# zyc-123/InstanceDiff

Measured on AMD Instinct MI355X. Metric: denoising steps/sec (256x256 bs16), higher is better.
Workload: dtype f32; 1 GPU; 256x256 1-ch synthetic, 1000-step reverse chain, batch 16 per GPU, 2 UNet fwd + reverse update per step; global_batch=16, parallelism=replicas x1 (no collective)

## Files before the change

instancediff_amd/csrc/conv_args.h:

```cpp
#pragma once
#include "common.h"

namespace idiff_detail {

struct GnTail {
    const float* gamma;
    const float* beta;
    const float* film;
    long long film_ld;
    float eps;
    int groups;
    float* out_a;
    float* out_b;
    float* mean_rstd;
};

struct ConvArgs {
    const float* src0;
    const float* src1;
    long long bs0, bs1;
    int C0v, C1v;
    int C0r;
    int Cin;
    int B, Hin, Win, Hout, Wout;
    int Cout;
    const float* wpk;
    const float* wwino;
    const float* wwino4;
    const float* bias;
    const float* pro_a;
    const float* pro_b;
    float* out;
    long long obs;
    const float* res;
    long long rbs;
    const float* vec;
    const float* aux;
    long long abs_;
    const float* aux_a;
    const float* aux_b;
    float* stats;
    GnTail gn;
    int tiles_x, ntiles, ncob;
    unsigned total_wg;
};

bool conv_wino_eligible(const ConvArgs& a, int ks, int mode);
int launch_conv_wino(const ConvArgs& a, int mode, hipStream_t st);

long long conv_wino4_items(const ConvArgs& a, int ks, int mode, bool requested = false);
int launch_conv_wino4(const ConvArgs& a, int mode, hipStream_t st);
int launch_conv_wino4h(const ConvArgs& a, int mode, hipStream_t st);

bool conv1x1_x3_eligible(const ConvArgs& a, int mode);
int launch_conv1x1_x3(const ConvArgs& a, int mode, const void* wx3, hipStream_t st);

bool conv_bf16_eligible(const ConvArgs& a, int ks, int mode, const void* wbf16);
int launch_conv_bf16(const ConvArgs& a, int mode, const void* wbf16, hipStream_t st);

}
```

instancediff_amd/csrc/conv_igemm.hip:

```cpp
#include <stdlib.h>

#include <type_traits>

#include "conv_args.h"

using idiff_detail::ConvArgs;

namespace {

typedef float floatx2 __attribute__((ext_vector_type(2)));

template <int KS, int CK, int TWL, int MODE, bool VECW, int MB, int SPEC>
__global__ __launch_bounds__(256) void conv_igemm_kernel(const ConvArgs a) {
    constexpr int BM = 32 * MB;
    constexpr int TW = 1 << TWL;
    constexpr int TH = 256 / TW;
    constexpr int PAD = KS / 2;
    constexpr int TRH = TH + KS - 1;
    constexpr int RS = TW + KS - 1;
    constexpr int PS = TRH * RS;
    constexpr int IN_TILE = ((CK * PS + 3) / 4) * 4;
    constexpr int TAPS = KS * KS;
    constexpr int W_TILE = TAPS * CK * BM;
    constexpr int BUF = IN_TILE + W_TILE;
// ... 466 lines not shown
        if (KS == 3 && MODE == IDIFF_CONV_NORMAL && MB == 2 && vecw) {
            if (a.pro_a) return launch_conv<KS, CK, 5, MODE, true, MB, 2>(a, st);
            if (a.src1) return launch_conv<KS, CK, 5, MODE, true, MB, 3>(a, st);
            return launch_conv<KS, CK, 5, MODE, true, MB, 1>(a, st);
        }
        return vecw ? launch_conv<KS, CK, 5, MODE, true, MB, 0>(a, st) : launch_conv<KS, CK, 5, MODE, false, MB, 0>(a, st);
    }
    if (twl == 4) return vecw ? launch_conv<KS, CK, 4, MODE, true, MB, 0>(a, st) : launch_conv<KS, CK, 4, MODE, false, MB, 0>(a, st);
    return vecw ? launch_conv<KS, CK, 3, MODE, true, MB, 0>(a, st) : launch_conv<KS, CK, 3, MODE, false, MB, 0>(a, st);
}

template <int KS, int CK, int MODE>
int dispatch_mb(const ConvArgs& a, int twl, int mb, bool vecw, hipStream_t st) {
    return mb == 2 ? dispatch_tw<KS, CK, MODE, 2>(a, twl, vecw, st) : dispatch_tw<KS, CK, MODE, 1>(a, twl, vecw, st);
}

inline int pick_twl(int Wout) { return Wout >= 24 ? 5 : (Wout >= 16 ? 4 : 3); }

__global__ void pack_weight_kernel(const float* __restrict__ w, float* __restrict__ out, int Cout, int Cin, int taps, int transpose) {
    const long long n = (long long)Cout * Cin * taps;
    for (long long i = blockIdx.x * (long long)blockDim.x + threadIdx.x; i < n; i += (long long)gridDim.x * blockDim.x) {
        if (!transpose) {
            const int co = i % Cout;
            const int ci = (i / Cout) % Cin;
            const int tap = i / ((long long)Cout * Cin);
            out[i] = w[((long long)co * Cin + ci) * taps + tap];
        } else {
            const int ci = i % Cin;
            const int co = (i / Cin) % Cout;
            const int tap = i / ((long long)Cout * Cin);
            out[i] = w[((long long)co * Cin + ci) * taps + (taps - 1 - tap)];
        }
    }
}

}

static thread_local int g_last_algo = IDIFF_CONV_ALGO_DIRECT;
extern "C" int idiff_conv2d_last_algo(void) { return g_last_algo; }

extern "C" int idiff_conv2d_num_tiles(int Hout, int Wout) {
    const int twl = pick_twl(Wout);
    const int TW = 1 << twl, TH = 256 / TW;
    return ((Wout + TW - 1) / TW) * ((Hout + TH - 1) / TH);
}

static int conv2d_run(const idiff_conv_desc* d, idiff_stream_t stream, const bool plan) {
    IDIFF_CHECK_ARG(d && d->src0 && d->wpk && d->out, "conv2d: null pointer");
    IDIFF_CHECK_ARG(d->B > 0 && d->C0 > 0 && d->Cout > 0 && d->Hin > 0 && d->Win > 0, "conv2d: bad dims");
    IDIFF_CHECK_ARG(d->ks == 1 || d->ks == 3 || d->ks == 7, "conv2d: ks must be 1, 3 or 7 (got %d)", d->ks);
    IDIFF_CHECK_ARG(d->mode >= 0 && d->mode <= 2, "conv2d: bad mode %d", d->mode);
    IDIFF_CHECK_ARG((d->C1 > 0) == (d->src1 != nullptr), "conv2d: src1/C1 mismatch");
    IDIFF_CHECK_ARG(!(d->pro_a && d->C1 > 0), "conv2d: prologue needs a single source");
    IDIFF_CHECK_ARG((d->pro_a == nullptr) == (d->pro_b == nullptr), "conv2d: pro_a/pro_b must both be set");
    IDIFF_CHECK_ARG(!d->aux || (d->aux_a && d->aux_b), "conv2d: aux needs aux_a/aux_b");
    ConvArgs a;
    a.src0 = d->src0;
    a.src1 = d->src1;
    a.bs0 = d->src0_bstride;
    a.bs1 = d->src1_bstride;
    a.B = d->B;
    a.C0r = d->C0;
    a.Hin = d->Hin;
    a.Win = d->Win;
    a.Cout = d->Cout;
    a.wpk = d->wpk;
    a.wwino = d->wwino;
    a.wwino4 = d->wwino4;
    a.bias = d->bias;
    a.pro_a = d->pro_a;
    a.pro_b = d->pro_b;
    a.out = d->out;
    a.obs = d->out_bstride;
    a.res = d->res;
    a.rbs = d->res_bstride;
    a.vec = d->vec;
    a.aux = d->aux;
    a.abs_ = d->aux_bstride;
    a.aux_a = d->aux_a;
    a.aux_b = d->aux_b;
    a.stats = d->stats;
    memset(&a.gn, 0, sizeof(a.gn));
    const bool want_gn = d->gn_out_a != nullptr;
    if (want_gn) {
        IDIFF_CHECK_ARG(d->stats && d->gn_out_b && d->gn_groups > 0 && d->Cout % d->gn_groups == 0 && d->Cout / d->gn_groups <= 256,
                        "conv2d: GroupNorm finalize needs stats, gn_out_b and groups dividing Cout (<= 256 channels per group)");
        a.gn.gamma = d->gn_gamma, a.gn.beta = d->gn_beta, a.gn.film = d->gn_film, a.gn.film_ld = d->gn_film_ld, a.gn.eps = d->gn_eps;
        a.gn.groups = d->gn_groups, a.gn.out_a = d->gn_out_a, a.gn.out_b = d->gn_out_b, a.gn.mean_rstd = d->gn_mean_rstd;
    }
    auto finalize_after = [&](int rc) -> int {
        if (rc != IDIFF_OK || !want_gn) return rc;
        return idiff_gn_finalize(d->stats, a.ntiles, a.B, a.Cout, d->gn_groups, a.Hout * a.Wout, d->gn_gamma, d->gn_beta, d->gn_film, d->gn_film_ld,
                                 d->gn_eps, d->gn_out_a, d->gn_out_b, d->gn_mean_rstd, stream);
    };
    if (d->mode == IDIFF_CONV_UNSHUFFLE2) {
        IDIFF_CHECK_ARG(d->ks == 1 && d->C1 == 0, "conv2d: unshuffle mode needs ks=1 and a single source");
        IDIFF_CHECK_ARG(d->Hin % 2 == 0 && d->Win % 2 == 0, "conv2d: unshuffle needs even H, W");
        a.C0v = d->C0 * 4;
        a.C1v = 0;
        a.Hout = d->Hin / 2;
        a.Wout = d->Win / 2;
    } else if (d->mode == IDIFF_CONV_UPSAMPLE2) {
        a.C0v = d->C0;
        a.C1v = d->C1;
        a.Hout = d->Hin * 2;
        a.Wout = d->Win * 2;
    } else {
        a.C0v = d->C0;
        a.C1v = d->C1;
        a.Hout = d->Hin;
        a.Wout = d->Win;
    }
    a.Cin = a.C0v + a.C1v;
    IDIFF_CHECK_ARG(a.bs0 >= (long long)d->C0 * d->Hin * d->Win, "conv2d: src0_bstride too small");
    IDIFF_CHECK_ARG(d->C1 == 0 || a.bs1 >= (long long)d->C1 * d->Hin * d->Win, "conv2d: src1_bstride too small");
    IDIFF_CHECK_ARG(a.obs >= (long long)d->Cout * a.Hout * a.Wout, "conv2d: out_bstride too small");
    int twl = pick_twl(a.Wout);
    const int mb = a.Cout <= 32 ? 1 : 2;
    const bool vecw = (a.Cout % 4 == 0) && ((reinterpret_cast<uintptr_t>(a.wpk) & 15) == 0);
    const bool in16 = (reinterpret_cast<uintptr_t>(a.src0) & 15) == 0 && (reinterpret_cast<uintptr_t>(a.src1) & 15) == 0 && a.bs0 % 4 == 0 &&
                      (!a.src1 || a.bs1 % 4 == 0);
    if (d->ks == 1 && d->mode == IDIFF_CONV_NORMAL && !a.stats && mb == 2 && vecw && in16 && ((long long)a.Hout * a.Wout) % 256 == 0 &&
        a.Wout >= 32) {
        a.Win = a.Wout = a.Hout * a.Wout;
        a.Hin = a.Hout = 1;
        twl = 8;
    }
    const int TW = 1 << twl, TH = 256 / TW;
    const int bm = 32 * mb;
    a.tiles_x = (a.Wout + TW - 1) / TW;
    a.ntiles = a.tiles_x * ((a.Hout + TH - 1) / TH);
    a.ncob = (a.Cout + bm - 1) / bm;
    const long long total = (long long)a.B * a.ntiles * a.ncob;
    IDIFF_CHECK_ARG(total < (1ll << 31), "conv2d: grid too large");
    a.total_wg = (unsigned)total;
    hipStream_t st = (hipStream_t)stream;
    const bool hard = d->algo_request > 0;
    const int req = (hard ? d->algo_request : -d->algo_request) - 1;
    IDIFF_CHECK_ARG(req == -1 || req == IDIFF_CONV_ALGO_DIRECT || req == IDIFF_CONV_ALGO_WINOGRAD || req == IDIFF_CONV_ALGO_WINOGRAD4 ||
                        req == IDIFF_CONV_ALGO_WINOGRAD4H || req == IDIFF_CONV_ALGO_X3 || req == IDIFF_CONV_ALGO_BF16,
                    "conv2d: bad algo_request %d", d->algo_request);
    IDIFF_CHECK_ARG(d->operands == 0 || d->operands == 1, "conv2d: bad operands %d", d->operands);
    {
        const bool reqbf = req == IDIFF_CONV_ALGO_BF16;
        const bool can = idiff_detail::conv_bf16_eligible(a, d->ks, d->mode, d->wbf16);
        IDIFF_CHECK_ARG(!(hard && reqbf) || can, "conv2d: algo_request bf16 but the layer is not a 3x3 that tiles for it (Cout %% 64, C0 / C1 %% 32, "
                        "Hout %% 8, Wout %% 32) or has no bf16 image");
        if (can && (reqbf || (req == -1 && d->operands == 1))) {
            g_last_algo = IDIFF_CONV_ALGO_BF16;
            if (plan) return IDIFF_OK;
            return finalize_after(idiff_detail::launch_conv_bf16(a, d->mode, d->wbf16, st));
        }
    }
    {
        static const bool x3_on = [] {
            const char* e = getenv("IDIFF_X3");
            return !e || atoi(e) != 0;
        }();
        const bool reqx3 = req == IDIFF_CONV_ALGO_X3;
        bool can = false;
        ConvArgs ax = a;
        if (d->ks == 1 && d->wx3 != nullptr && (reinterpret_cast<uintptr_t>(d->wx3) & 15) == 0) {
            if (d->mode == IDIFF_CONV_NORMAL) {
                can = twl == 8 && idiff_detail::conv1x1_x3_eligible(ax, d->mode);
            } else if (d->mode == IDIFF_CONV_UNSHUFFLE2) {
                ax.ncob = a.Cout / 64;
                ax.ntiles = (int)(((long long)a.Hout * a.Wout) / 256);
                ax.tiles_x = ax.ntiles;
                const long long tot = (long long)a.B * ax.ntiles * ax.ncob;
                ax.total_wg = (unsigned)tot;
                can = tot > 0 && tot < (1ll << 31) && idiff_detail::conv1x1_x3_eligible(ax, d->mode);
            }
        }
        IDIFF_CHECK_ARG(!(hard && reqx3) || can, "conv2d: algo_request bf16x3 but the layer is not a 1x1 that tiles by 256 pixels with a split weight image");
        if (can && (reqx3 || (req == -1 && x3_on))) {
            g_last_algo = IDIFF_CONV_ALGO_X3;
            if (plan) return IDIFF_OK;
            return idiff_detail::launch_conv1x1_x3(ax, d->mode, d->wx3, st);
        }
    }
    static const int w4h_mode = [] {
        const char* e = getenv("IDIFF_W4H");
        return e ? atoi(e) : 1;
    }();
    const bool req4 = req == IDIFF_CONV_ALGO_WINOGRAD4, req4h = req == IDIFF_CONV_ALGO_WINOGRAD4H;
    const long long items16 = (req == -1 || req4 || req4h) ? idiff_detail::conv_wino4_items(a, d->ks, d->mode, req4 || req4h) : 0;
    if (items16 > 0) {
        const long long items8 = (long long)a.ntiles * a.ncob;
        const bool w4_ok = a.Cin >= 16;
        IDIFF_CHECK_ARG(!(hard && req4) || w4_ok, "conv2d: algo_request F(4x4,3x3) 16x32-item kernel needs Cin >= 16 (got %d)", a.Cin);
        bool half;
        if (req4h) half = true;
        else if (req4 && w4_ok) half = false;
        else if (items16 >= 16 && w4_ok) half = w4h_mode == 2 || (w4h_mode == 3 && a.src1 != nullptr);
        else half = w4h_mode >= 1 && items8 >= 16;
        if (half) {
            g_last_algo = IDIFF_CONV_ALGO_WINOGRAD4H;
            if (plan) return IDIFF_OK;
            return finalize_after(idiff_detail::launch_conv_wino4h(a, d->mode, st));
        }
        if (w4_ok && (req4 || items16 >= 16)) {
            g_last_algo = IDIFF_CONV_ALGO_WINOGRAD4;
            if (plan) return IDIFF_OK;
            return finalize_after(idiff_detail::launch_conv_wino4(a, d->mode, st));
        }
    }
    IDIFF_CHECK_ARG(!hard || !(req4 || req4h), "conv2d: algo_request F(4x4,3x3) but the shape does not tile for it");
    if ((req == -1 || req == IDIFF_CONV_ALGO_WINOGRAD || !hard) && req != IDIFF_CONV_ALGO_DIRECT && idiff_detail::conv_wino_eligible(a, d->ks, d->mode)) {
        g_last_algo = IDIFF_CONV_ALGO_WINOGRAD;
        if (plan) return IDIFF_OK;
        return finalize_after(idiff_detail::launch_conv_wino(a, d->mode, st));
    }
    IDIFF_CHECK_ARG(!hard || req != IDIFF_CONV_ALGO_WINOGRAD, "conv2d: algo_request F(2x2,3x3) but the shape does not tile for it");
    g_last_algo = IDIFF_CONV_ALGO_DIRECT;
    if (plan) {
        IDIFF_CHECK_ARG(!(d->ks == 1 && d->mode == IDIFF_CONV_UPSAMPLE2), "conv2d: upsample mode needs ks=3");
        IDIFF_CHECK_ARG(d->ks != 7 || d->mode == IDIFF_CONV_NORMAL, "conv2d: ks=7 needs normal mode");
        return IDIFF_OK;
    }
    if (d->ks == 3) {
        if (d->mode == IDIFF_CONV_NORMAL) return finalize_after(dispatch_mb<3, 8, IDIFF_CONV_NORMAL>(a, twl, mb, vecw, st));
        return finalize_after(dispatch_mb<3, 8, IDIFF_CONV_UPSAMPLE2>(a, twl, mb, vecw, st));
    }
    if (d->ks == 1) {
        IDIFF_CHECK_ARG(d->mode != IDIFF_CONV_UPSAMPLE2, "conv2d: upsample mode needs ks=3");
        if (d->mode == IDIFF_CONV_NORMAL) return finalize_after(dispatch_mb<1, 16, IDIFF_CONV_NORMAL>(a, twl, mb, vecw, st));
        return finalize_after(dispatch_mb<1, 16, IDIFF_CONV_UNSHUFFLE2>(a, twl, mb, vecw, st));
    }
    IDIFF_CHECK_ARG(d->mode == IDIFF_CONV_NORMAL, "conv2d: ks=7 needs normal mode");
    return finalize_after(dispatch_mb<7, 2, IDIFF_CONV_NORMAL>(a, twl, mb, vecw, st));
}

extern "C" int idiff_conv2d_fwd(const idiff_conv_desc* d, idiff_stream_t stream) { return conv2d_run(d, stream, false); }

extern "C" int idiff_conv2d_plan(const idiff_conv_desc* d) {
    const int keep = g_last_algo;
    const int rc = conv2d_run(d, nullptr, true);
    const int algo = g_last_algo;
    g_last_algo = keep;
    return rc != IDIFF_OK ? rc : algo;
}

static int pack_common(const float* w, float* wpk, int Cout, int Cin, int ks, int tr, idiff_stream_t stream) {
    IDIFF_CHECK_ARG(w && wpk && Cout > 0 && Cin > 0 && ks > 0, "pack_conv_weight: bad args");
    const long long n = (long long)Cout * Cin * ks * ks;
    const int grid = (int)((n + 255) / 256 > 4096 ? 4096 : (n + 255) / 256);
    hipLaunchKernelGGL(pack_weight_kernel, dim3(grid), dim3(256), 0, (hipStream_t)stream, w, wpk, Cout, Cin, ks * ks, tr);
    IDIFF_CHECK_LAUNCH("pack_conv_weight");
    return IDIFF_OK;
}
extern "C" int idiff_pack_conv_weight(const float* w, float* wpk, int Cout, int Cin, int ks, idiff_stream_t stream) {
    return pack_common(w, wpk, Cout, Cin, ks, 0, stream);
}
extern "C" int idiff_pack_conv_weight_T(const float* w, float* wpk, int Cout, int Cin, int ks, idiff_stream_t stream) {
    return pack_common(w, wpk, Cout, Cin, ks, 1, stream);
}
```

instancediff_amd/ops.py:

```python
import contextlib
import ctypes as C
import math
import os
import threading

import torch

from . import _lib
from ._lib import ConvDesc, check

CONV_NORMAL, CONV_UPSAMPLE2, CONV_UNSHUFFLE2 = 0, 1, 2
ACT_NONE, ACT_SILU, ACT_GELU = 0, 1, 2
SDE_STEP, SDE_MEAN, SDE_ODE = 0, 1, 2

PROFILE = None
ALGO_TRACE = None
WGRAD_TRACE = None


def launch_count():
    return int(_lib.load().idiff_launch_count())


def _stream():
    return C.c_void_p(torch.cuda.current_stream().cuda_stream)


def _p(t):
    return None if t is None else C.c_void_p(t.data_ptr())


def _chk(t, name="tensor", dtype=torch.float32):
    if t is None:
        return
    if not t.is_cuda:
        raise _lib.IdiffError(f"{name} must live on the GPU (the hot path has no CPU fallback)")
    if t.dtype != dtype:
        raise _lib.IdiffError(f"{name} must be {dtype}, got {t.dtype}")


def _bs(t, name="tensor"):
    _chk(t, name)
    exp = 1
    for d in range(t.dim() - 1, 0, -1):
        if t.shape[d] != 1 and t.stride(d) != exp:
            raise _lib.IdiffError(f"{name}: samples must be contiguous (shape {tuple(t.shape)}, strides {t.stride()})")
        exp *= t.shape[d]
    return t.stride(0) if t.shape[0] > 1 else max(exp, t.stride(0))


def _c(t, name="tensor", dtype=torch.float32):
    _chk(t, name, dtype)
    if t is not None and not t.is_contiguous():
        raise _lib.IdiffError(f"{name} must be contiguous")
    return t


WINOGRAD = bool(int(os.environ.get("IDIFF_WINOGRAD", "1")))
X3 = bool(int(os.environ.get("IDIFF_X3", "1")))
WINOGRAD4 = WINOGRAD and bool(int(os.environ.get("IDIFF_WINOGRAD4", "1")))
WINOGRAD4_DGRAD = bool(int(os.environ.get("IDIFF_WINOGRAD4_DGRAD", "1")))


CONV_ALGO_DIRECT, CONV_ALGO_WINOGRAD, CONV_ALGO_STREAM1X1, CONV_ALGO_WINOGRAD4, CONV_ALGO_WINOGRAD4H, CONV_ALGO_X3 = 0, 1, 2, 3, 4, 5
CONV_ALGO_BF16 = 6
_ALGO_REQUEST = threading.local()
CONV_OPERANDS = ("f32", "bf16")
_OPERANDS = threading.local()


@contextlib.contextmanager
def conv_operands(kind):
    if kind not in CONV_OPERANDS:
        raise ValueError(f"conv operands must be one of {CONV_OPERANDS}, got {kind!r}")
    old = getattr(_OPERANDS, "kind", "f32")
    _OPERANDS.kind = kind
    try:
        yield
    finally:
        _OPERANDS.kind = old


def current_conv_operands():
    return getattr(_OPERANDS, "kind", "f32")


@contextlib.contextmanager
def request_conv3x3_algo(algo):
    old = getattr(_ALGO_REQUEST, "algo", None)
    _ALGO_REQUEST.algo = algo
    try:
        yield
    finally:
        _ALGO_REQUEST.algo = old


def _alloc_conv_images(w, transpose, bf16=False):
    lib = _lib.load()
    _c(w, "weight")
    co, ci, k, _ = w.shape
    out = torch.empty((k * k, co, ci) if transpose else (k * k, ci, co), device=w.device, dtype=torch.float32)
    if bf16 and k == 3:
        out.bf16 = torch.empty((lib.idiff_conv_weight_bf16_bytes(co, ci, 1 if transpose else 0) // 2,), device=w.device, dtype=torch.int16)
    if k == 3 and WINOGRAD and co % 8 == 0 and ci % 8 == 0 and (ci if transpose else co) % 16 == 0:
        cconv, kconv = (ci, co) if transpose else (co, ci)
        out.wino = torch.empty((16 * kconv * ((cconv + 63) // 64) * 64,), device=w.device, dtype=torch.float32)
        if WINOGRAD4 and (WINOGRAD4_DGRAD or not transpose):
            out.wino4 = torch.empty((36 * kconv * ((cconv + 63) // 64) * 64,), device=w.device, dtype=torch.float32)
    cconv1, kconv1 = (ci, co) if transpose else (co, ci)
    if k == 1 and X3 and cconv1 % 64 == 0 and kconv1 >= 32 and kconv1 % 8 == 0:
        out.x3 = torch.empty((lib.idiff_conv1x1_x3_image_bytes(cconv1, kconv1) // 2,), device=w.device, dtype=torch.int16)
    return out


def _fill_conv_images(out, w, transpose, algo=None):
    lib = _lib.load()
    co, ci, k, _ = w.shape
    tr = 1 if transpose else 0
    if algo is None or algo == CONV_ALGO_DIRECT:
        fn = lib.idiff_pack_conv_weight_T if transpose else lib.idiff_pack_conv_weight
        check(fn(_p(w), _p(out), co, ci, k, _stream()), "pack_conv_weight")
    if hasattr(out, "wino") and (algo is None or algo == CONV_ALGO_WINOGRAD):
        check(lib.idiff_pack_conv_weight_wino(_p(w), _p(out.wino), co, ci, tr, _stream()), "pack_conv_weight_wino")
    if hasattr(out, "wino4") and (algo is None or algo in (CONV_ALGO_WINOGRAD4, CONV_ALGO_WINOGRAD4H)):
        check(lib.idiff_pack_conv_weight_wino4(_p(w), _p(out.wino4), co, ci, tr, _stream()), "pack_conv_weight_wino4")
    if hasattr(out, "x3") and (algo is None or algo == CONV_ALGO_X3):
        cconv1, kconv1 = (ci, co) if transpose else (co, ci)
        wm = w.reshape(co, ci).t().contiguous() if transpose else w
        check(lib.idiff_pack_conv1x1_x3(_p(wm), out.x3.data_ptr(), cconv1, kconv1, _stream()), "pack_conv1x1_x3")
    if hasattr(out, "bf16") and (algo is None or algo == CONV_ALGO_BF16):
        check(lib.idiff_pack_conv_weight_bf16(_p(w), out.bf16.data_ptr(), co, ci, tr, _stream()), "pack_conv_weight_bf16")


def pack_conv_weight(w, transpose=False, bf16=False):
    out = _alloc_conv_images(w, transpose, bf16)
    _fill_conv_images(out, w, transpose)
    return out


class LazyConvWeight:

    def __init__(self, w, transpose=False):
        self.w, self.transpose = _c(w, "weight"), transpose


def conv2d(src0, wpk, bias, ks, Cout, src1=None, mode=CONV_NORMAL, pro=None, out=None, res=None, vec=None, aux=None,
           want_stats=False, algo=None, gn=None, operands=None):
    lib = _lib.load()
    B, C0, Hin, Win = src0.shape
    operands = current_conv_operands() if operands is None else operands
    if operands not in CONV_OPERANDS:
        raise ValueError(f"conv operands must be one of {CONV_OPERANDS}, got {operands!r}")
    bf16 = operands == "bf16" and ks == 3
    lazy = wpk if isinstance(wpk, LazyConvWeight) else None
    if lazy is not None:
        wpk = _alloc_conv_images(lazy.w, lazy.transpose, bf16 or algo == CONV_ALGO_BF16)
    d = ConvDesc()
    if bf16:
        d.operands = 1
    wb = getattr(wpk, "bf16", None)
    if wb is not None and ks == 3:
        d.wbf16 = wb.data_ptr()
    if algo is not None:
        d.algo_request = 1 + algo
    elif ks == 3 and getattr(_ALGO_REQUEST, "algo", None) is not None:
        d.algo_request = -(1 + _ALGO_REQUEST.algo)
    d.src0, d.src0_bstride, d.C0 = src0.data_ptr(), _bs(src0, "src0"), C0
    if src1 is not None:
        assert src1.shape[0] == B and src1.shape[2:] == src0.shape[2:]
        d.src1, d.src1_bstride, d.C1 = src1.data_ptr(), _bs(src1, "src1"), src1.shape[1]
    d.B, d.Hin, d.Win, d.mode, d.ks, d.Cout = B, Hin, Win, mode, ks, Cout
    _c(wpk, "wpk")
    d.wpk = wpk.data_ptr()
    wino = getattr(wpk, "wino", None)
    if wino is not None and ks == 3:
        d.wwino = wino.data_ptr()
        wino4 = getattr(wpk, "wino4", None)
        if wino4 is not None:
            d.wwino4 = wino4.data_ptr()
    x3 = getattr(wpk, "x3", None)
    if x3 is not None and ks == 1 and mode in (CONV_NORMAL, CONV_UNSHUFFLE2):
        d.wx3 = x3.data_ptr()
    if bias is not None:
        d.bias = _c(bias, "bias").data_ptr()
    if pro is not None:
        d.pro_a, d.pro_b = _c(pro[0], "pro_a").data_ptr(), _c(pro[1], "pro_b").data_ptr()
    if mode == CONV_UPSAMPLE2:
        Hout, Wout = Hin * 2, Win * 2
    elif mode == CONV_UNSHUFFLE2:
        Hout, Wout = Hin // 2, Win // 2
    else:
        Hout, Wout = Hin, Win
    if out is None:
        out = torch.empty((B, Cout, Hout, Wout), device=src0.device, dtype=torch.float32)
    else:
        assert tuple(out.shape) == (B, Cout, Hout, Wout), (out.shape, (B, Cout, Hout, Wout))
    d.out, d.out_bstride = out.data_ptr(), _bs(out, "out")
    if res is not None:
        assert res.shape == out.shape
        d.res, d.res_bstride = res.data_ptr(), _bs(res, "res")
    if vec is not None:
        assert tuple(vec.shape) == (B, Cout)
        d.vec = _c(vec, "vec").data_ptr()
    if aux is not None:
        t, a, b = aux
        assert t.shape == out.shape
        d.aux, d.aux_bstride = t.data_ptr(), _bs(t, "aux")
        d.aux_a, d.aux_b = _c(a, "aux_a").data_ptr(), _c(b, "aux_b").data_ptr()
    stats = None
    bufs = gn.get("bufs") if gn is not None else None
    if want_stats or gn is not None:
        nt = lib.idiff_conv2d_num_tiles(Hout, Wout)
        stats = bufs[0] if bufs is not None else torch.empty((B, nt, Cout, 2), device=src0.device, dtype=torch.float32)
        assert tuple(stats.shape) == (B, nt, Cout, 2) and stats.is_contiguous() and stats.dtype == torch.float32
        d.stats = stats.data_ptr()
    gn_out = None
    if gn is not None:
        if bufs is not None:
            ga, gb = bufs[1], bufs[2]
            assert tuple(ga.shape) == (B, Cout) == tuple(gb.shape) and ga.is_contiguous() and gb.is_contiguous()
        else:
            ga, gb = torch.empty((B, Cout), device=src0.device, dtype=torch.float32), torch.empty((B, Cout), device=src0.device, dtype=torch.float32)
        d.gn_groups, d.gn_eps = int(gn["groups"]), float(gn.get("eps", 1e-5))
        d.gn_gamma, d.gn_beta = _c(gn["gamma"], "gn gamma").data_ptr(), _c(gn["beta"], "gn beta").data_ptr()
        film = gn.get("film")
        if film is not None:
            _chk(film, "film")
            assert film.shape[0] == B and film.shape[1] == 2 * Cout and film.stride(1) == 1
            d.gn_film, d.gn_film_ld = film.data_ptr(), film.stride(0)
        d.gn_out_a, d.gn_out_b = ga.data_ptr(), gb.data_ptr()
        gn_out = (ga, gb)
        if gn.get("want_mean_rstd"):
            mr = bufs[3] if bufs is not None else torch.empty((B, d.gn_groups, 2), device=src0.device, dtype=torch.float32)
            assert tuple(mr.shape) == (B, d.gn_groups, 2) and mr.is_contiguous()
            d.gn_mean_rstd = mr.data_ptr()
            gn_out = (ga, gb, mr)
    planned = None
    if lazy is not None:
        planned = lib.idiff_conv2d_plan(C.byref(d))
        check(min(planned, 0), "conv2d_plan")
        _fill_conv_images(wpk, lazy.w, lazy.transpose, planned)
    if PROFILE is not None:
        e0, e1 = torch.cuda.Event(enable_timing=True), torch.cuda.Event(enable_timing=True)
        e0.record()
        check(lib.idiff_conv2d_fwd(C.byref(d), _stream()), "conv2d_fwd")
        e1.record()
        Cin = (C0 * 4 if mode == CONV_UNSHUFFLE2 else C0) + (src1.shape[1] if src1 is not None else 0)
        PROFILE.append(dict(ks=ks, mode=mode, Cin=Cin, Cout=Cout, B=B, Hout=Hout, Wout=Wout, e0=e0, e1=e1, algo=lib.idiff_conv2d_last_algo(),
                            flops=2.0 * Cin * Cout * ks * ks * Hout * Wout * B))
    else:
        check(lib.idiff_conv2d_fwd(C.byref(d), _stream()), "conv2d_fwd")
    if planned is not None and lib.idiff_conv2d_last_algo() != planned:
        raise RuntimeError("conv2d: planned kernel %d, launched %d" % (planned, lib.idiff_conv2d_last_algo()))
    if ALGO_TRACE is not None:
        Cin = (C0 * 4 if mode == CONV_UNSHUFFLE2 else C0) + (src1.shape[1] if src1 is not None else 0)
        ALGO_TRACE[(lib.idiff_conv2d_last_algo(), ks, Cin, Cout, Hout, Wout)] += 1
    if gn is not None:
        return (out, gn_out, stats) if want_stats else (out, gn_out)
    return (out, stats) if want_stats else out


def gn_finalize(stats, groups, HW, gamma, beta, film=None, eps=1e-5, want_mean_rstd=False):
    lib = _lib.load()
    B, nt, Cc, _ = stats.shape
    a = torch.empty((B, Cc), device=stats.device, dtype=torch.float32)
    b = torch.empty_like(a)
    mr = torch.empty((B, groups, 2), device=stats.device, dtype=torch.float32) if want_mean_rstd else None
    film_ld = 0
    if film is not None:
        _chk(film, "film")
        assert film.shape[0] == B and film.shape[1] == 2 * Cc and film.stride(1) == 1
        film_ld = film.stride(0)
    check(lib.idiff_gn_finalize(_p(_c(stats)), nt, B, Cc, groups, HW, _p(_c(gamma)), _p(_c(beta)), _p(film), film_ld, eps,
                                _p(a), _p(b), _p(mr), _stream()), "gn_finalize")
    return (a, b, mr) if want_mean_rstd else (a, b)


def affine_silu_add(h, ab=None, res=None, vec=None, out=None):
    lib = _lib.load()
    B, Cc = h.shape[:2]
    HW = h.shape[2] * h.shape[3]
    if out is None:
        out = torch.empty(h.shape, device=h.device, dtype=torch.float32)
    a, b = ab if ab is not None else (None, None)
    check(lib.idiff_affine_silu_add(_p(h), _bs(h, "h"), _p(_c(a)), _p(_c(b)), _p(res), _bs(res, "res") if res is not None else 0,
                                    _p(_c(vec)), _p(out), _bs(out, "out"), B, Cc, HW, _stream()), "affine_silu_add")
    return out


def linear(x, w, bias=None, res=None, gscale=None, act_in=ACT_NONE, act_out=ACT_NONE, out=None):
    lib = _lib.load()
    _chk(x, "x"), _chk(w, "w")
    assert x.dim() == 2 and w.dim() == 2 and x.stride(1) == 1 and w.stride(1) == 1 and x.shape[1] == w.shape[1]
    R, K = x.shape
    N = w.shape[0]
    if out is None:
        out = torch.empty((R, N), device=x.device, dtype=torch.float32)
    assert out.stride(1) == 1 and tuple(out.shape) == (R, N)
    if res is not None:
        assert res.stride(1) == 1 and tuple(res.shape) == (R, N)
    check(lib.idiff_linear_fwd(_p(x), x.stride(0), _p(w), w.stride(0), _p(_c(bias)), _p(res), res.stride(0) if res is not None else 0,
                               _p(_c(gscale)), _p(out), out.stride(0), R, K, N, act_in, act_out, _stream()), "linear_fwd")
    return out


def linear_t(x, wT, bias=None, res=None, gscale=None, act_in=ACT_NONE, act_out=ACT_NONE, out=None, ln=None):
    lib = _lib.load()
    _chk(x, "x"), _chk(wT, "wT")
    assert x.dim() == 2 and wT.dim() == 2 and x.stride(1) == 1 and wT.stride(1) == 1 and x.shape[1] == wT.shape[0]
    R, K = x.shape
    N = wT.shape[1]
    if out is None:
        out = torch.empty((R, N), device=x.device, dtype=torch.float32)
    assert out.stride(1) == 1 and tuple(out.shape) == (R, N)
    if res is not None:
        assert res.stride(1) == 1 and tuple(res.shape) == (R, N)
    if ln is not None:
        assert act_in == ACT_NONE
        check(lib.idiff_linear_t_ln_fwd(_p(x), x.stride(0), _p(_c(ln[0])), _p(_c(ln[1])), float(ln[2]), _p(wT), wT.stride(0), _p(_c(bias)), _p(res),
                                        res.stride(0) if res is not None else 0, _p(_c(gscale)), _p(out), out.stride(0), R, K, N, act_out,
                                        _stream()), "linear_t_ln_fwd")
        return out
    check(lib.idiff_linear_t_fwd(_p(x), x.stride(0), _p(wT), wT.stride(0), _p(_c(bias)), _p(res), res.stride(0) if res is not None else 0,
                                 _p(_c(gscale)), _p(out), out.stride(0), R, K, N, act_in, act_out, _stream()), "linear_t_fwd")
    return out


def linear_t_grouped(groups):
    lib = _lib.load()
    n = len(groups)
    assert 1 <= n <= _lib.LINEAR_MAX_GROUPS, n
    arr = (_lib.LinearGroup * n)()
    outs = []
    for d, g in zip(arr, groups):
# ... 634 lines not shown
```

Before: 43.65 steps/s.

## Add bf16x3 MFMA kernel for thin-input 3x3 and 7x7 convolutions

Adds a new kernel for convolutions with few input channels (Cin<=8, e.g. the stem and output convs). The input is split into three bf16 parts held in LDS, taps are padded into the MFMA K dimension, and split-precision bf16 MFMAs reproduce fp32 accuracy. Weights stay in registers, and the kernel loops persistently over tiles with the next patch prefetched. It runs when such layers would otherwise fall back to the direct kernel, replacing scalar-FMA work on thin layers. In exchange it adds a packed weight image and more dispatch logic.

```diff
diff --git a/instancediff_amd/csrc/conv_args.h b/instancediff_amd/csrc/conv_args.h
--- a/instancediff_amd/csrc/conv_args.h
+++ b/instancediff_amd/csrc/conv_args.h
@@ -55,6 +55,10 @@
 bool conv1x1_x3_eligible(const ConvArgs& a, int mode);
 int launch_conv1x1_x3(const ConvArgs& a, int mode, const void* wx3, hipStream_t st);
 
+bool conv_thin_x3_eligible(const ConvArgs& a, int ks, int mode, const void* wx3);
+bool conv_thin_x3_preferred(const ConvArgs& a, int ks);
+int launch_conv_thin_x3(const ConvArgs& a, int ks, const void* wx3, hipStream_t st);
+
 bool conv_bf16_eligible(const ConvArgs& a, int ks, int mode, const void* wbf16);
 int launch_conv_bf16(const ConvArgs& a, int mode, const void* wbf16, hipStream_t st);
 
diff --git a/instancediff_amd/csrc/conv_igemm.hip b/instancediff_amd/csrc/conv_igemm.hip
--- a/instancediff_amd/csrc/conv_igemm.hip
+++ b/instancediff_amd/csrc/conv_igemm.hip
@@ -642,6 +642,7 @@
             return finalize_after(idiff_detail::launch_conv_bf16(a, d->mode, d->wbf16, st));
         }
     }
+    bool thin = false;
     {
         static const bool x3_on = [] {
             const char* e = getenv("IDIFF_X3");
@@ -662,11 +663,18 @@
                 can = tot > 0 && tot < (1ll << 31) && idiff_detail::conv1x1_x3_eligible(ax, d->mode);
             }
         }
-        IDIFF_CHECK_ARG(!(hard && reqx3) || can, "conv2d: algo_request bf16x3 but the layer is not a 1x1 that tiles by 256 pixels with a split weight image");
+        thin = x3_on || reqx3 ? idiff_detail::conv_thin_x3_eligible(a, d->ks, d->mode, d->wx3) : false;
+        IDIFF_CHECK_ARG(!(hard && reqx3) || can || thin,
+                        "conv2d: algo_request bf16x3 but the layer is neither a 1x1 that tiles by 256 pixels nor a thin-input 3x3 / 7x7, or has no split weight image");
         if (can && (reqx3 || (req == -1 && x3_on))) {
             g_last_algo = IDIFF_CONV_ALGO_X3;
             if (plan) return IDIFF_OK;
             return idiff_detail::launch_conv1x1_x3(ax, d->mode, d->wx3, st);
+        }
+        if (thin && reqx3) {
+            g_last_algo = IDIFF_CONV_ALGO_X3;
+            if (plan) return IDIFF_OK;
+            return idiff_detail::launch_conv_thin_x3(a, d->ks, d->wx3, st);
         }
     }
     static const int w4h_mode = [] {
@@ -702,6 +710,11 @@
         return finalize_after(idiff_detail::launch_conv_wino(a, d->mode, st));
     }
     IDIFF_CHECK_ARG(!hard || req != IDIFF_CONV_ALGO_WINOGRAD, "conv2d: algo_request F(2x2,3x3) but the shape does not tile for it");
+    if (thin && req != IDIFF_CONV_ALGO_DIRECT && idiff_detail::conv_thin_x3_preferred(a, d->ks)) {
+        g_last_algo = IDIFF_CONV_ALGO_X3;
+        if (plan) return IDIFF_OK;
+        return idiff_detail::launch_conv_thin_x3(a, d->ks, d->wx3, st);
+    }
     g_last_algo = IDIFF_CONV_ALGO_DIRECT;
     if (plan) {
         IDIFF_CHECK_ARG(!(d->ks == 1 && d->mode == IDIFF_CONV_UPSAMPLE2), "conv2d: upsample mode needs ks=3");
diff --git a/instancediff_amd/csrc/conv_thin_x3.hip b/instancediff_amd/csrc/conv_thin_x3.hip
--- /dev/null
+++ b/instancediff_amd/csrc/conv_thin_x3.hip
@@ -0,0 +1,283 @@
+#include <stdlib.h>
+
+#include "conv_args.h"
+
+using idiff_detail::ConvArgs;
+
+namespace {
+
+typedef unsigned uintx4 __attribute__((ext_vector_type(4)));
+typedef __bf16 bf16x8 __attribute__((ext_vector_type(8)));
+
+constexpr int NT = 256, TW = 32, TH_MAX = 16;
+constexpr int A_CHUNK = 12288;
+constexpr int A_PLSTR = 4096;
+
+struct ThinArgs {
+    const float* src0;
+    const float* src1;
+    long long bs0, bs1, obs;
+    const float* bias;
+    float* out;
+    const unsigned short* wx3;
+    int C0, Cin, H, W, Cout;
+    int TH, tiles_x, ntiles;
+    unsigned total;
+    int vec4;
+};
+
+template <typename T>
+__device__ __forceinline__ T* scalar_ptr(const T* p) {
+    const unsigned long long v = reinterpret_cast<unsigned long long>(p);
+    const unsigned lo = __builtin_amdgcn_readfirstlane((unsigned)v), hi = __builtin_amdgcn_readfirstlane((unsigned)(v >> 32));
+    return reinterpret_cast<T*>(((unsigned long long)hi << 32) | lo);
+}
+
+__device__ __forceinline__ floatx4 mma(const uintx4& a, const uintx4& b, const floatx4& c) {
+    return __builtin_amdgcn_mfma_f32_16x16x32_bf16(__builtin_bit_cast(bf16x8, a), __builtin_bit_cast(bf16x8, b), c, 0, 0, 0);
+}
+
+template <int KS>
+struct Geo {
+    static constexpr int KXP = KS == 7 ? 8 : 4;
+    static constexpr int SEGS = 8 / KXP;
+    static constexpr int PADL = KS / 2;
+    static constexpr int PWS = TW + KXP;
+    static constexpr int CIN_MAX = KS == 7 ? 2 : 8;
+    static constexpr int NE = (CIN_MAX * (TH_MAX + KS - 1) * PWS + NT - 1) / NT;
+};
+
+constexpr int RSRC_FLAGS = 0x00020000;
+constexpr unsigned OOB = 0x80000000u;
+
+template <int KS, int CBW, int KSTEPS>
+__global__ __launch_bounds__(NT) __attribute__((amdgpu_waves_per_eu(2, 2))) void conv_thin_x3_kernel(const ThinArgs a) {
+    using G = Geo<KS>;
+    constexpr int KXP = G::KXP, SEGS = G::SEGS, PADL = G::PADL, PWS = G::PWS, NE = G::NE;
+    extern __shared__ __attribute__((aligned(16))) unsigned char smem_raw[];
+
+    const int tid = threadIdx.x;
+    const int lane = tid & 63;
+    const int wave = __builtin_amdgcn_readfirstlane(tid >> 6);
+    const int n16 = lane & 15, kgl = lane >> 4;
+    const int ncg = (a.Cout >> 4) / CBW;
+    const int cog = wave % ncg, pg = wave / ncg, npg = 4 / ncg;
+    const int PH = a.TH + KS - 1;
+    const int nelem = a.Cin * PH * PWS;
+    const int plb = (nelem * 2 + 15) & ~15;
+    const long long HW = (long long)a.H * a.W;
+    const unsigned phmagic = (65536u + PH - 1) / PH;
+
+    uintx4 wreg[KSTEPS][CBW][3];
+    float biasv[CBW];
+    {
+        const int nchunks = (a.Cin * KS * KXP + 31) >> 5;
+        const __amdgpu_buffer_rsrc_t rw = __builtin_amdgcn_make_buffer_rsrc(scalar_ptr(a.wx3), 0, nchunks * A_CHUNK, RSRC_FLAGS);
+        const __amdgpu_buffer_rsrc_t rb = __builtin_amdgcn_make_buffer_rsrc(scalar_ptr(a.bias), 0, a.bias ? a.Cout * 4 : 0, RSRC_FLAGS);
+#pragma unroll
+        for (int cb = 0; cb < CBW; ++cb) {
+            const int co = (cog * CBW + cb) * 16 + n16;
+#pragma unroll
+            for (int ks = 0; ks < KSTEPS; ++ks)
+#pragma unroll
+                for (int p = 0; p < 3; ++p)
+                    wreg[ks][cb][p] = __builtin_bit_cast(uintx4, __builtin_amdgcn_raw_buffer_load_b128(rw, kgl * 1024 + co * 16, ks * A_CHUNK + p * A_PLSTR, 0));
+            biasv[cb] = __builtin_bit_cast(float, __builtin_amdgcn_raw_buffer_load_b32(rb, co * 4, 0, 0));
+        }
+    }
+
+    unsigned pk[NE];
+#pragma unroll
+    for (int i = 0; i < NE; ++i) {
+        const int idx = tid + i * NT;
+        const int c = idx % PWS, t = idx / PWS;
+        const int ci = (int)(((unsigned)t * phmagic) >> 16), rr = t - ci * PH;
+        pk[i] = idx < nelem ? (unsigned)(ci | (rr << 8) | (c << 16)) : 0xffffffffu;
+    }
+    const int ne = (nelem + NT - 1) / NT;
+    const bool two = a.src1 != nullptr;
+    unsigned xr[NE];
+    auto load_patch = [&](unsigned L) {
+        const bool live = L < a.total;
+        const unsigned Lc = live ? L : 0;
+        const int b = Lc / a.ntiles, t = Lc % a.ntiles;
+        const int y0 = (t / a.tiles_x) * a.TH - PADL, x0 = (t % a.tiles_x) * TW - PADL;
+        const int C1 = a.Cin - a.C0;
+        const float* const p0 = a.src0 + (long long)b * a.bs0;
+        const float* const p1 = a.src1 ? a.src1 + (long long)b * a.bs1 : p0;
+        const int rec0 = live ? (int)(a.C0 * HW * 4) : 0, rec1 = (live && a.src1) ? (int)(C1 * HW * 4) : 0;
+        const __amdgpu_buffer_rsrc_t r0 = __builtin_amdgcn_make_buffer_rsrc(scalar_ptr(p0), 0, __builtin_amdgcn_readfirstlane(rec0), RSRC_FLAGS);
+        const __amdgpu_buffer_rsrc_t r1 = __builtin_amdgcn_make_buffer_rsrc(scalar_ptr(p1), 0, __builtin_amdgcn_readfirstlane(rec1), RSRC_FLAGS);
+#pragma unroll
+        for (int i = 0; i < NE; ++i) {
+            if (i >= ne) break;
+            const int ci = pk[i] & 0xff, y = y0 + (int)((pk[i] >> 8) & 0xff), x = x0 + (int)((pk[i] >> 16) & 0xff);
+            const bool in = pk[i] != 0xffffffffu && (unsigned)y < (unsigned)a.H && (unsigned)x < (unsigned)a.W;
+            const bool first = ci < a.C0;
+            const unsigned o = (unsigned)(((first ? ci : ci - a.C0) * a.H + y) * a.W + x) * 4u;
+            unsigned v = __builtin_bit_cast(unsigned, __builtin_amdgcn_raw_buffer_load_b32(r0, (int)((in && first) ? o : OOB), 0, 0));
+            if (two)
+                v |= __builtin_bit_cast(unsigned, __builtin_amdgcn_raw_buffer_load_b32(r1, (int)((in && !first) ? o : OOB), 0, 0));
+            xr[i] = v;
+        }
+    };
+    auto stage = [&]() {
+#pragma unroll
+        for (int i = 0; i < NE; ++i) {
+            if (i >= ne) break;
+            const int idx = tid + i * NT;
+            if (idx < nelem) {
+                const unsigned u1 = xr[i];
+                const float r1 = __builtin_bit_cast(float, u1) - __builtin_bit_cast(float, u1 & 0xffff0000u);
+                const unsigned u2 = __builtin_bit_cast(unsigned, r1);
+                const float r2 = r1 - __builtin_bit_cast(float, u2 & 0xffff0000u);
+                const unsigned u3 = __builtin_bit_cast(unsigned, r2);
+                unsigned short* const d = reinterpret_cast<unsigned short*>(smem_raw) + idx;
+                d[0] = (unsigned short)(u1 >> 16);
+                d[plb >> 1] = (unsigned short)(u2 >> 16);
+                d[plb] = (unsigned short)(u3 >> 16);
+            }
+        }
+    };
+
+    int rowoff[KSTEPS][SEGS];
+#pragma unroll
+    for (int ks = 0; ks < KSTEPS; ++ks)
+#pragma unroll
+        for (int h = 0; h < SEGS; ++h) {
+            const int r = (ks * 4 + kgl) * SEGS + h;
+            const int ci = r / KS, ky = r % KS;
+            rowoff[ks][h] = (r < a.Cin * KS ? (ci * PH + ky) * (PWS / 2) : 0) + (n16 >> 1);
+        }
+    const unsigned sh = (n16 & 1) * 16;
+    const unsigned* const lds = reinterpret_cast<const unsigned*>(smem_raw);
+    const int plw = plb >> 2;
+
+    load_patch(blockIdx.x);
+    for (unsigned L = blockIdx.x; L < a.total; L += gridDim.x) {
+        __syncthreads();
+        stage();
+        __syncthreads();
+        load_patch(L + gridDim.x);
+        const int b = L / a.ntiles, t = L % a.ntiles;
+        const int y0 = (t / a.tiles_x) * a.TH, x0 = (t % a.tiles_x) * TW;
+        float* const outb = a.out + (long long)b * a.obs;
+        for (int ty = pg; ty < a.TH; ty += npg) {
+            const int y = y0 + ty;
+            if (y >= a.H) break;
+            floatx4 acc[2][CBW];
+#pragma unroll
+            for (int xb = 0; xb < 2; ++xb)
+#pragma unroll
+                for (int cb = 0; cb < CBW; ++cb) acc[xb][cb] = floatx4{0.f, 0.f, 0.f, 0.f};
+            const unsigned* const row = lds + ty * (PWS / 2);
+#pragma unroll
+            for (int ks = 0; ks < KSTEPS; ++ks) {
+                uintx4 av[2][3];
+#pragma unroll
+                for (int xb = 0; xb < 2; ++xb)
+#pragma unroll
+                    for (int p = 0; p < 3; ++p) {
+                        unsigned o[4];
+#pragma unroll
+                        for (int h = 0; h < SEGS; ++h) {
+                            const unsigned* const s = row + p * plw + rowoff[ks][h] + xb * 8;
+                            unsigned d[KXP / 2 + 1];
+#pragma unroll
+                            for (int i = 0; i <= KXP / 2; ++i) d[i] = s[i];
+#pragma unroll
+                            for (int i = 0; i < KXP / 2; ++i) o[h * (KXP / 2) + i] = __builtin_amdgcn_alignbit(d[i + 1], d[i], sh);
+                        }
+                        av[xb][p] = uintx4{o[0], o[1], o[2], o[3]};
+                    }
+#define IDIFF_THIN_MMA(PA, PB)                                                                        \
+    _Pragma("unroll") for (int cb = 0; cb < CBW; ++cb) _Pragma("unroll") for (int xb = 0; xb < 2; ++xb) \
+        acc[xb][cb] = mma(av[xb][PA], wreg[ks][cb][PB], acc[xb][cb]);
+                IDIFF_THIN_MMA(0, 2)
+                IDIFF_THIN_MMA(1, 1)
+                IDIFF_THIN_MMA(2, 0)
+                IDIFF_THIN_MMA(0, 1)
+                IDIFF_THIN_MMA(1, 0)
+                IDIFF_THIN_MMA(0, 0)
+#undef IDIFF_THIN_MMA
+            }
+#pragma unroll
+            for (int cb = 0; cb < CBW; ++cb) {
+                const int co = (cog * CBW + cb) * 16 + n16;
+                float* const orow = outb + (long long)co * HW + (long long)y * a.W;
+#pragma unroll
+                for (int xb = 0; xb < 2; ++xb) {
+                    const int x = x0 + 16 * xb + 4 * kgl;
+                    const floatx4 v = acc[xb][cb] + biasv[cb];
+                    if (a.vec4) {
+                        if (x < a.W) *reinterpret_cast<floatx4*>(orow + x) = v;
+                    } else {
+#pragma unroll
+                        for (int r = 0; r < 4; ++r)
+                            if (x + r < a.W) orow[x + r] = v[r];
+                    }
+                }
+            }
+        }
+    }
+}
+
+template <int KS, int CBW, int KSTEPS>
+int launch_one(const ThinArgs& t, int grid, size_t lds, hipStream_t st) {
+    hipLaunchKernelGGL((conv_thin_x3_kernel<KS, CBW, KSTEPS>), dim3(grid), dim3(NT), lds, st, t);
+    IDIFF_CHECK_LAUNCH("conv2d_fwd(thin x3)");
+    return IDIFF_OK;
+}
+
+int kxp_of(int ks) { return ks == 7 ? 8 : 4; }
+
+}
+
+namespace idiff_detail {
+
+bool conv_thin_x3_eligible(const ConvArgs& a, int ks, int mode, const void* wx3) {
+    if (mode != IDIFF_CONV_NORMAL || (ks != 3 && ks != 7) || !wx3 || (reinterpret_cast<uintptr_t>(wx3) & 15)) return false;
+    if (a.Cin > 8 || a.Cin * ks * kxp_of(ks) > 128 || (a.Cout != 16 && a.Cout != 32 && a.Cout != 64)) return false;
+    if (a.pro_a || a.stats || a.gn.out_a || a.res || a.vec || a.aux) return false;
+    const long long hw = (long long)a.Hout * a.Wout;
+    if (a.Hin != a.Hout || a.Win != a.Wout || hw * 8 * 4 >= (1ll << 31)) return false;
+    const long long tiles = (long long)((a.Wout + TW - 1) / TW) * ((a.Hout + 3) / 4) * a.B;
+    return tiles < (1ll << 31);
+}
+
+bool conv_thin_x3_preferred(const ConvArgs& a, int ks) {
+    const long long hw = (long long)a.Hout * a.Wout;
+    return !(ks == 3 && hw >= 64 * 64 && hw < 128 * 128);
+}
+
+int launch_conv_thin_x3(const ConvArgs& a, int ks, const void* wx3, hipStream_t st) {
+    ThinArgs t;
+    t.src0 = a.src0, t.src1 = a.src1, t.bs0 = a.bs0, t.bs1 = a.bs1, t.obs = a.obs;
+    t.bias = a.bias, t.out = a.out, t.wx3 = static_cast<const unsigned short*>(wx3);
+    t.C0 = a.C0v, t.Cin = a.Cin, t.H = a.Hout, t.W = a.Wout, t.Cout = a.Cout;
+    const long long hw = (long long)a.Hout * a.Wout;
+    t.TH = hw >= 128 * 128 ? 16 : 4;
+    t.tiles_x = (a.Wout + TW - 1) / TW;
+    t.ntiles = t.tiles_x * ((a.Hout + t.TH - 1) / t.TH);
+    t.total = (unsigned)((long long)a.B * t.ntiles);
+    t.vec4 = a.Wout % 4 == 0 && (reinterpret_cast<uintptr_t>(a.out) & 15) == 0 && a.obs % 4 == 0;
+    static std::atomic<int> cus[64];
+    int dev = 0, ncu = 0;
+    if (hipGetDevice(&dev) != hipSuccess) IDIFF_FAIL(IDIFF_E_HIP, "conv2d(thin x3): hipGetDevice");
+    if (dev >= 0 && dev < 64) ncu = cus[dev].load(std::memory_order_relaxed);
+    if (ncu <= 0) {
+        if (hipDeviceGetAttribute(&ncu, hipDeviceAttributeMultiprocessorCount, dev) != hipSuccess || ncu <= 0)
+            IDIFF_FAIL(IDIFF_E_HIP, "conv2d(thin x3): no compute-unit count");
+        if (dev >= 0 && dev < 64) cus[dev].store(ncu, std::memory_order_relaxed);
+    }
+    const int grid = (int)(t.total < 2u * ncu ? t.total : 2u * ncu);
+    const int kxp = kxp_of(ks);
+    const int nelem = a.Cin * (t.TH + ks - 1) * (TW + kxp);
+    const size_t lds = 3 * (size_t)((nelem * 2 + 15) & ~15);
+    const int ncb = a.Cout / 16;
+    if (ks == 7) return ncb == 1 ? launch_one<7, 1, 4>(t, grid, lds, st) : launch_one<7, 2, 4>(t, grid, lds, st);
+    if (a.Cin * 3 * kxp <= 64) return ncb == 1 ? launch_one<3, 1, 2>(t, grid, lds, st) : launch_one<3, 2, 2>(t, grid, lds, st);
+    return ncb == 1 ? launch_one<3, 1, 3>(t, grid, lds, st) : launch_one<3, 2, 3>(t, grid, lds, st);
+}
+
+}
diff --git a/instancediff_amd/ops.py b/instancediff_amd/ops.py
--- a/instancediff_amd/ops.py
+++ b/instancediff_amd/ops.py
@@ -110,7 +110,14 @@
     cconv1, kconv1 = (ci, co) if transpose else (co, ci)
     if k == 1 and X3 and cconv1 % 64 == 0 and kconv1 >= 32 and kconv1 % 8 == 0:
         out.x3 = torch.empty((lib.idiff_conv1x1_x3_image_bytes(cconv1, kconv1) // 2,), device=w.device, dtype=torch.int16)
-    return out
+    if thin_x3_taps(co, ci, k) and X3 and not transpose:
+        out.x3 = torch.empty((lib.idiff_conv1x1_x3_image_bytes(co, ci * k * thin_x3_taps(co, ci, k)) // 2,), device=w.device, dtype=torch.int16)
+    return out
+
+
+def thin_x3_taps(co, ci, k):
+    taps = {3: 4, 7: 8}.get(k, 0)
+    return taps if taps and ci <= 8 and ci * k * taps <= 128 and co in (16, 32, 64) else 0
 
 
 def _fill_conv_images(out, w, transpose, algo=None):
@@ -125,8 +132,13 @@
     if hasattr(out, "wino4") and (algo is None or algo in (CONV_ALGO_WINOGRAD4, CONV_ALGO_WINOGRAD4H)):
         check(lib.idiff_pack_conv_weight_wino4(_p(w), _p(out.wino4), co, ci, tr, _stream()), "pack_conv_weight_wino4")
     if hasattr(out, "x3") and (algo is None or algo == CONV_ALGO_X3):
-        cconv1, kconv1 = (ci, co) if transpose else (co, ci)
-        wm = w.reshape(co, ci).t().contiguous() if transpose else w
+        if k == 1:
+            cconv1, kconv1 = (ci, co) if transpose else (co, ci)
+            wm = w.reshape(co, ci).t().contiguous() if transpose else w
+        else:
+            taps = thin_x3_taps(co, ci, k)
+            cconv1, kconv1 = co, ci * k * taps
+            wm = torch.nn.functional.pad(w, (0, taps - k)).contiguous()
         check(lib.idiff_pack_conv1x1_x3(_p(wm), out.x3.data_ptr(), cconv1, kconv1, _stream()), "pack_conv1x1_x3")
     if hasattr(out, "bf16") and (algo is None or algo == CONV_ALGO_BF16):
         check(lib.idiff_pack_conv_weight_bf16(_p(w), out.bf16.data_ptr(), co, ci, tr, _stream()), "pack_conv_weight_bf16")
@@ -179,7 +191,7 @@
         if wino4 is not None:
             d.wwino4 = wino4.data_ptr()
     x3 = getattr(wpk, "x3", None)
-    if x3 is not None and ks == 1 and mode in (CONV_NORMAL, CONV_UNSHUFFLE2):
+    if x3 is not None and ((ks == 1 and mode in (CONV_NORMAL, CONV_UNSHUFFLE2)) or (ks in (3, 7) and mode == CONV_NORMAL)):
         d.wx3 = x3.data_ptr()
     if bias is not None:
         d.bias = _c(bias, "bias").data_ptr()
```

After: 43.99 steps/s (median of 6 runs). No clear change (+0.8%).
